# xipengwang/AprilSAM

Measured on AMD Instinct MI355X. Metric: Gauss-Newton iterations/sec + factorise ms on M3500 (chi2 match <=1e-6), higher is better.
Workload: dtype f64; 1 GPU; M3500 batch april_graph_cholesky, 1 replica per GPU (3500 poses, 5454 factors, n=10500); parallelism=single GPU, fronts=680, levels=9, nnz_L=422121

## Files before the change

### aprilsam_amd/csrc/kernels.hip.h

```cpp
#pragma once
#include <hip/hip_runtime.h>
#include <stdint.h>

#include <type_traits>
namespace asam {

constexpr int PROF_SLOTS = 16;
constexpr int PROF_XCD_UP = 12, PROF_XCD_DN = 13;
constexpr int PROF_X_STORED = 14, PROF_X_DRAINED = 11, PROF_X_FLAG = 15;
constexpr int PROF_EA_ISSUED = 8, PROF_EA_DATA = 9, PROF_EA_ADDS = 10, PROF_EA_REST = 14, PROF_EA_END = 15;
#ifdef APRILSAM_AMD_EA_STAMPS
constexpr bool EA_STAMPS = true;
#else
constexpr bool EA_STAMPS = false;
#endif
__device__ __forceinline__ int xcc_id() { return __builtin_amdgcn_s_getreg(20 | (0 << 6) | ((4 - 1) << 11)) & 7; }
constexpr int TPB = 256;
constexpr int NB = 32;
constexpr int TILE = 64;
constexpr int ASM_CB = 4;
constexpr int OBP = 4;

struct FrontDesc {
    long long off;
    int nsb, nub, first;
    int dest_begin, dest_end;
    int ch_begin, ch_end;
    int rows_begin;
    int parent;
    int dinv0;
    int prim1, prim2;
    int own_nw;
    int pad;
};
static_assert(sizeof(FrontDesc) == 64, "FrontDesc must stay one cache line");
struct DestRec { int brow, bcol, src_begin, src_end; };
struct ChildRec {
    long long uoff;
    int cR;
    int cnu;
    int rel_begin;
    int pad;
};
static_assert(sizeof(ChildRec) == 24, "ChildRec layout");

struct DevPlan {
    int nF;
    const FrontDesc *fd;
    const DestRec *dest;
    const ChildRec *child;
    const int *f_rows, *f_rel;
    const int *f_own; int own_lo, own_hi;
    const int *slot_blk, *slot_rhs;
    const int *src_idx;
    const double *lambda;
    long long *prof;
    int prof_mode;
    int schur_first_nub;
    int *epoch; const int *flevel; int l0; const int *marks;
    int xmode; uint4 *xg; unsigned xg_bytes;
};
enum { X_FLUSH = 0, X_WT = 1, X_TAGGED = 2 };
constexpr int XG_CONST = -1;

__host__ __device__ inline int asm_chunks(int nbc) { return (nbc + ASM_CB - 1) / ASM_CB; }
struct SyrkRange { int k_lo, k_hi, col_lo, col_hi, ntr, ntc; };
__host__ __device__ inline SyrkRange syrk_range(int R, int C, int ns, int s_lo, int s_hi, int tile = TILE, bool ahead = false) {
    SyrkRange g;
    g.k_lo = s_lo * NB;
    g.k_hi = s_hi * NB < ns ? s_hi * NB : ns;
    g.col_lo = g.k_hi;
    g.col_hi = ahead ? (g.k_hi + OBP * NB < ns ? g.k_hi + OBP * NB : ns) : C;
    if (g.k_hi <= g.k_lo || g.col_hi <= g.col_lo) { g.ntr = g.ntc = 0; return g; }
    g.ntr = ((R - 2) - g.col_lo + tile - 1) / tile;
    g.ntc = (g.col_hi - g.col_lo + tile - 1) / tile;
    return g;
}
__host__ __device__ inline int syrk_tiles(int R, int C, int ns, int s_lo, int s_hi, int tile = TILE, bool ahead = false) {
    SyrkRange g = syrk_range(R, C, ns, s_lo, s_hi, tile, ahead);
    return g.ntc * g.ntr - g.ntc * (g.ntc - 1) / 2;
}
__device__ __forceinline__ int find_seg(const int *__restrict__ pre, int n, int bid) {
    int lo = 0, hi = n;
    while (hi - lo > 1) { int m = (lo + hi) >> 1; if (pre[m] <= bid) lo = m; else hi = m; }
    return lo;
}

__device__ __forceinline__ void trapezoid_tile(int l, int ntr, int ntc, int *ti, int *tj_);
constexpr int SYRK_SB = 8;
constexpr int SYRK_MODE_XCD_SHIFT = 8;
__host__ __device__ inline void trapezoid_tile_xcd(int l, int nt, int ntr, int ntc, int *ti, int *tj) {
// ... 742 lines not shown
    for (int l = wave; l < ntiles; l += nw) {
        int ti = l, tj = 0;
        while (ti >= ntr - tj) { ti -= ntr - tj; tj++; }
        ti += tj;
        const int i0 = col_lo + 16 * ti, j0 = col_lo + 16 * tj;
        const int rj = min(j0 + l15, Rv - 1), ri = min(i0 + l15, Rv - 1);
        const int i = i0 + l15, jb = j0 + l4;
        const int cbase = jb * ld + i;
        bool ok[4];
#pragma unroll
        for (int reg = 0; reg < 4; reg++) { const int j = jb + 4 * reg; ok[reg] = i < Rv && j < col_hi && i >= j; }
        double cv[4], x[4], y[4];
#pragma unroll
        for (int reg = 0; reg < 4; reg++) cv[reg] = S[ok[reg] ? cbase + 4 * reg * ld : 0];
#pragma unroll
        for (int ks = 0; ks < 4; ks++) {
            const int kk = 4 * ks + l4;
            const double *col = S + (k_lo + (kk < kw ? kk : 0)) * ld;
            x[ks] = col[rj]; y[ks] = col[ri];
        }
        d4_t acc = (d4_t){ 0, 0, 0, 0 };
#pragma unroll
        for (int ks = 0; ks < 4; ks++) {
            if (ks < nk) {
                const bool kok = 4 * ks + l4 < kw;
                acc = __builtin_amdgcn_mfma_f64_16x16x4f64(kok ? x[ks] : 0.0, kok ? y[ks] : 0.0, acc, 0, 0, 0);
            }
        }
#pragma unroll
        for (int reg = 0; reg < 4; reg++) if (ok[reg]) S[cbase + 4 * reg * ld] = cv[reg] - acc[reg];
    }
}

constexpr int GB = 4;

constexpr int BW = 16;
template <int NT, int BWT>
__device__ __forceinline__ void chain_block(double *S, int ld, int k0, int wdt, int Rv, int *bad, double (&Dd)[BWT], int nwc) {
    constexpr int BROWS = 64 - BWT;
    constexpr int PER = BWT <= 8 ? 1 : (BWT - 2 + 7) / 8;
    const int wave = __builtin_amdgcn_readfirstlane(threadIdx.x >> 6), lane = threadIdx.x & 63;
    const bool isdiag = lane < BWT;
    const int below0 = k0 + wdt;
    const int nchunk = max(1, (Rv - below0 + BROWS - 1) / BROWS);
    if (wave >= nchunk) return;
    for (int ch = wave + ((nchunk - 1 - wave) / nwc) * nwc; ch >= wave; ch -= nwc) {
        const int row = isdiag ? k0 + lane : below0 + BROWS * ch + (lane - BWT);
        const bool valid = isdiag ? lane < wdt : row < Rv;
        const int rowc = valid ? row : k0;
        double D[BWT];
#pragma unroll
        for (int c = 0; c < BWT; c++) D[c] = S[(size_t)(k0 + (c < wdt ? c : 0)) * ld + rowc];
        int isbad = 0;
        double dn = readlane_d(D[0], 0);
        if (!(dn > 0)) isbad = 1;
        double inv = fast_rsqrt(dn);
#pragma unroll
        for (int j = 0; j < BWT; j++) {
            D[j] *= inv;
            double lc[BWT];
            if (j + 1 < BWT) {
                lc[j + 1] = readlane_d(D[j], j + 1);
                D[j + 1] = fma(-D[j], lc[j + 1], D[j + 1]);
                dn = readlane_d(D[j + 1], j + 1);
                if (j + 1 < wdt && !(dn > 0)) isbad = 1;
            }
// ... 8 lines not shown
                    else if (st == 1 || st == 4) e = -h * y;
                    else if (st == 2 || st == 5) e = fma(e, y, 0.5);
                    else if (st == 3 || st == 6) y = fma(y, e, y);
                }
#pragma unroll
                for (int q = 0; q < PER; q++) {
                    const int c = j + 2 + PER * st + q;
                    if (c < BWT) D[c] = fma(-D[j], lc[c], D[c]);
                }
                __builtin_amdgcn_sched_barrier(0);
            }
            inv = y;
        }
        if (valid && !isdiag) {
#pragma unroll
            for (int c = BWT - 1; c >= 0; c--) S[(size_t)(k0 + (c < wdt ? c : 0)) * ld + row] = (c < wdt) ? D[c] : D[0];
        }
        if (ch == 0) {
#pragma unroll
            for (int c = 0; c < BWT; c++) Dd[c] = D[c];
            if (isbad && lane == 0) { if (atomicCAS(bad, 0, 1) == 0) { bad[2] = 1; bad[3] = k0 / 3; } }
        }
    }
}
template <int BWT>
__device__ __forceinline__ void chain_store_diag(double *S, int ld, int k0, int wdt, const double (&Dd)[BWT]) {
    const int r = threadIdx.x & 63;
    if (r < wdt) {
#pragma unroll
        for (int c = 0; c < BWT; c++) if (c < wdt) S[(k0 + c) * ld + k0 + r] = (c <= r) ? Dd[c] : 0.0;
    }
}
template <int NT>
__device__ __forceinline__ void factor_dense_blk(double *S, int ld, int ns, int Rv, int hi, int *bad, double * , long long *pf = nullptr) {
    constexpr int NW = NT / 64;
    long long t_chain = 0, t_syrk = 0, t0 = 0;
    const int wave = __builtin_amdgcn_readfirstlane(threadIdx.x >> 6);
    auto chain_sync_store = [&](int k0, int nwc) {
        const int wdt = min(BW, ns - k0);
        if (wdt <= 8) {
            double D8[8];
            chain_block<NT, 8>(S, ld, k0, wdt, Rv, bad, D8, nwc);
            __syncthreads();
            if (wave == 0) chain_store_diag<8>(S, ld, k0, wdt, D8);
        } else {
            double D16[16];
            chain_block<NT, 16>(S, ld, k0, wdt, Rv, bad, D16, nwc);
            __syncthreads();
            if (wave == 0) chain_store_diag<16>(S, ld, k0, wdt, D16);
        }
    };
    auto chain_waves = [&](int k0) {
        const int wdt = min(BW, ns - k0), brows = 64 - (wdt <= 8 ? 8 : 16);
        const int nchunk = max(1, (Rv - (k0 + wdt) + brows - 1) / brows);
        return min(nchunk, NW / 2);
    };
    if (pf) t0 = wall_clock64();
    chain_sync_store(0, NW);
    if (pf) { const long long t1 = wall_clock64(); t_chain += t1 - t0; t0 = t1; }
    for (int k0 = 0; k0 < ns; k0 += BW) {
        const int wdt = min(BW, ns - k0), below0 = k0 + wdt;
        if (below0 < ns) {
            const int next_hi = min(below0 + BW, ns), cw = chain_waves(below0);
            if (NW >= 8) lds_syrk16<NT>(S, ld, k0, below0, below0, next_hi, Rv, 1, NW - 1);
            else lds_syrk16<NT>(S, ld, k0, below0, below0, next_hi, Rv);
            __syncthreads();
            if (pf) { const long long t1 = wall_clock64(); t_syrk += t1 - t0; t0 = t1; }
            if (wave < cw) {
                long long w0_ = 0, c0_ = 0;
                if (pf) { w0_ = wall_clock64(); c0_ = clock64(); }
                chain_sync_store(below0, cw);
                if (pf && threadIdx.x == 0) { pf[10] += clock64() - c0_; pf[15] += wall_clock64() - w0_; }
            } else {
                if (next_hi < hi) lds_syrk16<NT>(S, ld, k0, below0, next_hi, hi, Rv, cw, NW - cw);
                __syncthreads();
            }
            if (pf) { const long long t1 = wall_clock64(); t_chain += t1 - t0; t0 = t1; }
        } else {
            __syncthreads();
            if (below0 < hi) lds_syrk16<NT>(S, ld, k0, below0, below0, hi, Rv);
            __syncthreads();
            if (pf) { const long long t1 = wall_clock64(); t_syrk += t1 - t0; t0 = t1; }
        }
    }
    if (pf && threadIdx.x == 0) { pf[8] = t_chain; pf[9] = t_syrk; }
}
template <int NT>
__device__ __forceinline__ void factor_front_blk(double *S, int ld, int nsb, int nbc, int *bad, double *stage, int nbc_upd = -1, long long *pf = nullptr) {
    if (nbc_upd < 0) nbc_upd = nbc;
    factor_dense_blk<NT>(S, ld, 3 * nsb, 3 * (nbc + 1) - 2, 3 * nbc_upd, bad, stage, pf);
}

__host__ __device__ inline size_t small_front_lds(int R, int C, int nw) { return (size_t)(R | 1) * C * 8 + wl_bytes(nw); }
__host__ __device__ inline size_t panel_front_lds(int R, int ns, int nw) { return (size_t)(R | 1) * ns * 8 + wl_bytes(nw); }
__host__ __device__ inline bool front_runs_full(int R, int C, int nw, long long full_lds_limit) { return (long long)small_front_lds(R, C, nw) <= full_lds_limit; }

template <int NT>
__device__ __forceinline__ void front_small_body(const DevPlan &P, const int t, double *__restrict__ pool, const double *__restrict__ Hc, int *bad,
                                                 long long full_lds_limit, int *flags, int wait, double *S) {
    const int *wflags = wait ? flags : nullptr;
    const int ev = flags ? flag_value(P) : 0;
    const FrontDesc D = P.fd[t];
    const int nsb = D.nsb, nbc = D.nsb + D.nub;
    const int R = 3 * (nbc + 1), C = 3 * nbc, ld = R | 1;
    double *Fg = pool + D.off;
    if (P.prof && threadIdx.x == 0) P.prof[(size_t)t * PROF_SLOTS + PROF_XCD_UP] = 1 + xcc_id();
    if (front_runs_full(R, C, NT / 64, full_lds_limit)) {
        int2 *wl = (int2 *)(S + (size_t)ld * C);
        if (P.prof && threadIdx.x == 0) P.prof[(size_t)t * PROF_SLOTS + 0] = wall_clock64();
        assemble_front<NT, ASM_LDS>(P, D, pool, Hc, 0, nbc, true, S, ld, nullptr, 0, wl, P.prof ? P.prof + (size_t)t * PROF_SLOTS : nullptr, wflags, bad, ev);
        if (P.prof && threadIdx.x == 0) P.prof[(size_t)t * PROF_SLOTS + 1] = wall_clock64();
        factor_front_blk<NT>(S, ld, nsb, nbc, bad, (double *)wl, -1, (P.prof && (!EA_STAMPS || P.prof_mode < 4)) ? P.prof + (size_t)t * PROF_SLOTS : nullptr);
        if (P.prof && threadIdx.x == 0) P.prof[(size_t)t * PROF_SLOTS + 2] = wall_clock64();
        for (int c = 3 * nsb + (threadIdx.x >> 6); c < C; c += NT / 64) {
            int r0 = 3 * (c / 3);
            for (int r = r0 + (threadIdx.x & 63); r < R; r += 64) Fg[(size_t)c * R + r] = S[(size_t)c * ld + r];
        }
        if (flags) publish_flag(flags + t, ev);
        for (int c = threadIdx.x >> 6; c < 3 * nsb; c += NT / 64) {
            int r0 = 3 * (c / 3);
            for (int r = r0 + (threadIdx.x & 63); r < R; r += 64) Fg[(size_t)c * R + r] = S[(size_t)c * ld + r];
        }
    } else {
        const int ns = 3 * nsb;
        int2 *wl = (int2 *)(S + (size_t)ld * ns);
        const bool schur_first = P.schur_first_nub > 0 && D.nub >= P.schur_first_nub;
        if (P.prof && threadIdx.x == 0) P.prof[(size_t)t * PROF_SLOTS + 0] = wall_clock64();
        if (schur_first) assemble_front<NT, ASM_SPLIT>(P, D, pool, Hc, 0, nsb, false, S, ld, Fg, R, wl, P.prof ? P.prof + (size_t)t * PROF_SLOTS : nullptr, wflags, bad, ev);
        else assemble_front<NT, ASM_SPLIT>(P, D, pool, Hc, 0, nbc, true, S, ld, Fg, R, wl, P.prof ? P.prof + (size_t)t * PROF_SLOTS : nullptr, wflags, bad, ev);
        if (P.prof && threadIdx.x == 0) P.prof[(size_t)t * PROF_SLOTS + 1] = wall_clock64();
        factor_front_blk<NT>(S, ld, nsb, nbc, bad, (double *)wl, nsb, (P.prof && (!EA_STAMPS || P.prof_mode < 4)) ? P.prof + (size_t)t * PROF_SLOTS : nullptr);
        if (P.prof && threadIdx.x == 0) P.prof[(size_t)t * PROF_SLOTS + 2] = wall_clock64();
        if (schur_first) {
            lds_panel_syrk<NT, 2>(S, ld, 0, ns, ns, C, R - 2, Fg, R);
            __syncthreads();
            assemble_front<NT, ASM_GLOBAL, false>(P, D, pool, Hc, nsb, nbc, false, nullptr, 0, Fg, R, wl, nullptr, nullptr, bad);
        }
        else if (nbc > nsb) lds_panel_syrk<NT, 1>(S, ld, 0, ns, ns, C, R - 2, Fg, R);
        if (flags) publish_flag(flags + t, ev);
        for (int c = threadIdx.x >> 6; c < ns; c += NT / 64) {
            int r0 = 3 * (c / 3);
            for (int r = r0 + (threadIdx.x & 63); r < R; r += 64) Fg[(size_t)c * R + r] = S[(size_t)c * ld + r];
        }
    }
    if (P.prof) { __syncthreads(); if (threadIdx.x == 0) P.prof[(size_t)t * PROF_SLOTS + 3] = wall_clock64(); }
}
constexpr int UPD_MAXF = 4;
constexpr int UPD_MAXC = 4;
struct UpdRec {
    long long old_off;
    int mode;
    int old_nub;
    int wout;
    int mask;
    int n_own, own_f[UPD_MAXF], own_la[UPD_MAXF], own_lb[UPD_MAXF], own_slot[UPD_MAXF];
    int n_ch, ch_t[UPD_MAXC], ch_wout[UPD_MAXC], ch_rel[UPD_MAXC], ch_cnu[UPD_MAXC], ch_mask[UPD_MAXC];
    int pad[3];
};
static_assert(sizeof(UpdRec) == 192, "UpdRec layout");
struct UpdCtx {
    const UpdRec *recs;
    double *wbuf;
    int *wflags;
    const int *fa, *fb; const double *Z, *Wm, *lp, *st;
};
__host__ __device__ inline size_t update_front_lds(int R, int ns, int nact) {
    return (size_t)((size_t)ns * (R | 1) + (size_t)3 * nact * (R | 1) + 8 * ns + 3 * (ns | 1) + 16) * 8;
}
template <int NT>
__device__ __forceinline__ void front_update_body(const DevPlan &P, const int t, const UpdRec &rec, const UpdCtx &uc, double *__restrict__ pool,
                                                  int *flags, int *bad, double *S) {
    constexpr int NW = NT / 64;
// ... 1580 lines not shown
```

### aprilsam_amd/csrc/solver.h

```cpp
#pragma once
#include <vector>
#include "../../include/aprilsam_amd.h"

namespace asam {

struct Options {
    int leaf_nodes = 16;
    int deterministic = 0;
    int use_graph = 1;
    int device_timing = 0;
    int trust_factor_cache = 0;
    int small_lds_kb = 156;
    int inc_fast = 1;
    int inc_multi = 1;
    int inc_one = 1;
    int inc_one_up = 3, inc_one_dn = 4, inc_one_threads = 512, inc_one_spin = 1;
    int inc_tail = 1;
    int inc_inline = 1;
    int inc_tail_solve = 1;
    int inc_lazy_states = 1;
    int inc_replan_tall = 1;
    int inc_update = 1;
    int speculate_factors = 1;
    int warm_up = 1;
    int syrk_xcd_order = 512;
    int syrk_small_tiles = 320;
    int syrk_pair_tiles = 2048;
    int syrk_group = 3;
    int schur_first = 40;
    int small_threads = 1024;
    int tp_threads = 512;
    int tp_fronts = 1000;
    int tp_lds_kb = 80;
    int amalg = 0;
    int amalg_max = 64;
    int pin_last = 0;
    int batch_extend = 1;
    int extend_tail_fronts = 3;
    int persist = 1;
    int persist_max_fronts = 240;
    int persist_leaves = 1;
    int persist_up = 2;
    int xcd_place = 1;
    int asm_balance = 1;
    int tail_poses = 28;
    int blk_backsolve = 1;
    int wave_backsolve = 1;
    int tagged_x = 1;
    int linearize_staged_min = 32768;
    int mem_cap_mb = 0;
    int solve_chunk_cols = 0;
    int pool_guard = 0;
    int pool_poison = 0;
    int skip_flag_waits = 0;
    int polar_on_host = 0;
    int gaussian_on_host = 0;
    int panel_mode = 1;
};
extern Options g_opt;

void batch_step(april_graph_t *g, april_graph_cholesky_param_t *param);
void inc_step(april_graph_t *g, april_graph_cholesky_param_t *param);
void inc_solve_only(april_graph_t *g, april_graph_cholesky_param_t *param);
double graph_chi2(april_graph_t *g);
int batch_resident(april_graph_t *g, april_graph_cholesky_param_t *param, int iters, double *chi2_out, double *ms_out);
int resident_begin(april_graph_t *g, april_graph_cholesky_param_t *param);
int resident_steps(april_graph_t *g, april_graph_cholesky_param_t *param, int n, int mode);
int resident_sync(april_graph_t *g, april_graph_cholesky_param_t *param);
double resident_chi2(april_graph_t *g);
int resident_end(april_graph_t *g, april_graph_cholesky_param_t *param);
int level_profile(const april_graph_cholesky_param_t *param, double *out, int cap_levels);
int debug_front_forms(const april_graph_cholesky_param_t *param, int *out, int cap);
int debug_inc_forms(const april_graph_cholesky_param_t *param, int *out, int cap);
int kernel_profile(const april_graph_cholesky_param_t *param, double *ms, long long *calls, double *flops, double *bytes, const char **names);
void drop_context(const april_graph_cholesky_param_t *p);
void drop_graph_pack(const april_graph_t *g);
bool get_stats(const april_graph_cholesky_param_t *p, aprilsam_amd_stats_t *out);
// ... 73 lines not shown
```

### aprilsam_amd/csrc/solver.hip.cpp

```cpp
#include <hip/hip_runtime.h>
#include <rccl/rccl.h>
#include <dlfcn.h>

#include <algorithm>
#include <array>
#include <chrono>
#include <thread>
#include <cmath>
#include <cstdarg>
#include <cstdio>
#include <cstdlib>
#include <cstring>
#include <functional>
#include <map>
#include <memory>
#include <atomic>
#include <mutex>
#include <string>
#include <unordered_map>
#include <vector>

#include "../../include/aprilsam_amd.h"
#include "errors.h"
#include "kernels.hip.h"
// ... 19 lines not shown

#define HIPCHECK(expr)                                                                                 \
    do {                                                                                               \
        hipError_t e_ = (expr);                                                                        \
        if (e_ != hipSuccess) {                                                                        \
            (void)hipGetLastError();                                                                   \
            fail(e_ == hipErrorOutOfMemory ? ERR_OOM : ERR_HIP, "%s failed: %s (%s:%d)", #expr, hipGetErrorString(e_), __FILE__, __LINE__); \
        }                                                                                              \
    } while (0)

static double now_ms() {
    return std::chrono::duration<double, std::milli>(std::chrono::steady_clock::now().time_since_epoch()).count();
}

Options g_opt;
struct OptionDef { const char *name; int Options::*member; int min_value; bool policy; int max_value = 0x7fffffff; };
static const OptionDef OPTION_TABLE[] = {
    { "leaf_nodes", &Options::leaf_nodes, 1, false }, { "deterministic", &Options::deterministic, 0, true }, { "use_graph", &Options::use_graph, 0, true },
    { "device_timing", &Options::device_timing, 0, true }, { "trust_factor_cache", &Options::trust_factor_cache, 0, true },
    { "small_lds_kb", &Options::small_lds_kb, 0, false }, { "syrk_xcd_order", &Options::syrk_xcd_order, 0, false },
    { "schur_first", &Options::schur_first, 0, false }, { "syrk_small_tiles", &Options::syrk_small_tiles, 0, false }, { "syrk_pair_tiles", &Options::syrk_pair_tiles, 0, false }, { "syrk_group", &Options::syrk_group, 2, false, 8 }, { "panel_mode", &Options::panel_mode, 0, false },
    { "small_threads", &Options::small_threads, 64, false }, { "tp_fronts", &Options::tp_fronts, 0, false }, { "tp_lds_kb", &Options::tp_lds_kb, 0, false },
    { "tp_threads", &Options::tp_threads, 64, false }, { "inc_fast", &Options::inc_fast, 0, true }, { "inc_multi", &Options::inc_multi, 0, true },
    { "inc_one", &Options::inc_one, 0, true }, { "inc_one_up", &Options::inc_one_up, 1, true }, { "inc_one_dn", &Options::inc_one_dn, 1, true },
    { "inc_one_threads", &Options::inc_one_threads, 64, true }, { "inc_one_spin", &Options::inc_one_spin, 0, true }, { "inc_tail", &Options::inc_tail, 0, false },
    { "inc_inline", &Options::inc_inline, 0, true }, { "inc_update", &Options::inc_update, 0, true }, { "inc_tail_solve", &Options::inc_tail_solve, 0, true },
    { "inc_lazy_states", &Options::inc_lazy_states, 0, true }, { "inc_replan_tall", &Options::inc_replan_tall, 0, true },
    { "speculate_factors", &Options::speculate_factors, 0, true }, { "warm_up", &Options::warm_up, 0, true }, { "pin_last", &Options::pin_last, 0, false }, { "persist", &Options::persist, 0, false },
    { "persist_max_fronts", &Options::persist_max_fronts, 0, false }, { "xcd_place", &Options::xcd_place, 0, false }, { "persist_leaves", &Options::persist_leaves, 0, false, 1 }, { "persist_up", &Options::persist_up, 0, false, 3 }, { "linearize_staged_min", &Options::linearize_staged_min, 0, false },
    { "wave_backsolve", &Options::wave_backsolve, 0, false }, { "tagged_x", &Options::tagged_x, 0, false, 2 }, { "blk_backsolve", &Options::blk_backsolve, 0, false }, { "tail_poses", &Options::tail_poses, 8, false },
    { "batch_extend", &Options::batch_extend, 0, true }, { "extend_tail_fronts", &Options::extend_tail_fronts, 0, true }, { "mem_cap_mb", &Options::mem_cap_mb, 0, true }, { "solve_chunk_cols", &Options::solve_chunk_cols, 0, true },
    { "pool_guard", &Options::pool_guard, 0, false }, { "amalg", &Options::amalg, 0, false }, { "amalg_max", &Options::amalg_max, 1, false }, { "pool_poison", &Options::pool_poison, 0, false }, { "skip_flag_waits", &Options::skip_flag_waits, 0, false },
    { "polar_on_host", &Options::polar_on_host, 0, false, 1 }, { "gaussian_on_host", &Options::gaussian_on_host, 0, false, 1 }, { "asm_balance", &Options::asm_balance, 0, false, 1 },
};
static const OptionDef *find_option(const char *name) {
    for (const OptionDef &d : OPTION_TABLE) if (!strcmp(d.name, name)) return &d;
    return nullptr;
}
static std::once_flag g_opt_once;
static void load_env_options() {
    std::call_once(g_opt_once, [] {
        for (const OptionDef &d : OPTION_TABLE) {
            std::string env = "APRILSAM_AMD_";
            for (const char *q = d.name; *q; q++) env += (char)toupper((unsigned char)*q);
            const char *sv = getenv(env.c_str());
            if (sv && *sv) g_opt.*(d.member) = std::min(d.max_value, std::max(d.min_value, (int)atof(sv)));
        }
    });
}

constexpr int MAX_SLOTS = 64;
static std::atomic<int> g_device{ -1 };
static std::mutex g_slot_mu[MAX_SLOTS];
static thread_local int t_slot = 0;
static int device_count() {
    static std::atomic<int> cached{ 0 };
    int n = cached.load(std::memory_order_relaxed);
    if (n > 0) return n;
    if (hipGetDeviceCount(&n) != hipSuccess) { (void)hipGetLastError(); return 0; }
    if (n > 0) cached.store(n, std::memory_order_relaxed);
    return n;
}
static int physical_device(int slot) { const int n = device_count(); return n > 0 ? slot % n : 0; }
static thread_local int t_device = -1;
template <class V> struct Registry {
    using Map = std::map<const void *, std::unique_ptr<V>>;
// ... 413 lines not shown
```

### aprilsam_amd/csrc/solver_context.inc.h

```cpp
enum { K_LINEARIZE = 0, K_FRONT_SMALL, K_ASSEMBLE_BIG, K_PANEL_BIG, K_SYRK_BIG, K_BACKSOLVE, K_UPDATE, NKERN };
static const char *const KNAMES[NKERN] = { "k_linearize", "k_front_small", "k_assemble_big", "k_panel_big", "k_syrk_big", "k_backsolve", "k_update_states" };
struct Launch { int list_off, pre_off, n, grid; bool single = false; int tile = TILE; };

struct LevelPlan {
    int small_off = 0, n_small = 0; size_t small_lds = 0;
    long long full_limit = 0;
    int small_nt = 512;
    int n_big = 0; size_t asm_lds = 0;
    Launch asm_big{};
    std::vector<Launch> syrka, syrk1;
    bool paired = false;
    std::vector<Launch> bchain, btile, syrkw;
    int all_off = 0, n_all = 0; size_t solve_lds = 0;
    size_t solve_w_lds = 0; int maxns = 0;
    Launch bs_gemv{};
    Launch bs_blk{}; size_t bs_blk_lds = 0;
    int rest_off = 0, n_rest = 0; size_t rest_lds = 0;
};

struct IncState {
    bool ready = false;
    bool pristine = false;
    int Nb = 0, Fb = 0, nF0 = 0, nLev0 = 0;
    int cap_nodes = 0, cap_fact = 0;
// ... 507 lines not shown
    const double u1 = uprof ? now_ms() : 0;
    const bool inc = c.want_inc;
    const int INC_NODES_ = inc ? INC_NODES : 0, INC_FACT_ = inc ? INC_FACT : 0;
    const size_t INC_I32_ = inc ? INC_I32 : 0, INC_DEST_ = inc ? INC_DEST : 0, INC_CHILD_ = inc ? INC_CHILD : 0, INC_TAB_ = inc ? INC_TAB : 0;
    c.inc.cap_nodes = INC_NODES_; c.inc.cap_fact = INC_FACT_;
    std::vector<int> i32;
    auto put32 = [&](const std::vector<int> &v) { size_t o = i32.size(); i32.insert(i32.end(), v.begin(), v.end()); if (v.empty()) i32.push_back(0); return o; };
    size_t o_rows = put32(P.f_rows), o_rel = put32(P.f_rel);
    const bool own_tab = g_opt.asm_balance && !lay && !P.f_rel.empty();
    const size_t o_own = own_tab ? put32(std::vector<int>(P.f_rel.size(), -1)) : 0;
    size_t o_sb = put32(P.slot_blk); i32.resize(i32.size() + (size_t)3 * INC_FACT_, -1);
    size_t o_sr = put32(P.slot_rhs); i32.resize(i32.size() + (size_t)2 * INC_FACT_, -1);
    c.inc.i32_used = (long long)i32.size(); c.inc.dest_used = (long long)P.dest.size(); c.inc.child_used = (long long)P.ch_idx.size();
    for (int t = 0; t < P.nF; t++) fd[t].rows_begin = (int)(o_rows + P.f_rows_ptr[t]);
    for (size_t k = 0; k < P.ch_idx.size(); k++) ch[k].rel_begin = (int)(o_rel + P.f_rows_ptr[ch[k].pad]);
    c.d_i32.need(i32.size() + INC_I32_); c.d_fd.need(fd.size() + 1 + (inc ? MAX_TAIL_FRONTS : 0)); c.d_child.need(ch.size() + INC_CHILD_);
    c.d_dest.need(std::max<size_t>(1, P.dest.size()) + INC_DEST_);
    HIPCHECK(hipMemcpyAsync(c.d_i32.p, i32.data(), i32.size() * 4, hipMemcpyHostToDevice, s));
    HIPCHECK(hipMemcpyAsync(c.d_fd.p, fd.data(), fd.size() * sizeof(FrontDesc), hipMemcpyHostToDevice, s));
    HIPCHECK(hipMemcpyAsync(c.d_child.p, ch.data(), ch.size() * sizeof(ChildRec), hipMemcpyHostToDevice, s));
    static_assert(sizeof(DestRec) == sizeof(Plan::DestRec), "DestRec layout");
    if (!P.dest.empty()) HIPCHECK(hipMemcpyAsync(c.d_dest.p, P.dest.data(), P.dest.size() * sizeof(DestRec), hipMemcpyHostToDevice, s));
    c.d_lambda.need((size_t)P.N + INC_NODES_);
    DevPlan &d = c.dp;
    d.nF = P.nF;
    d.fd = c.d_fd.p; d.dest = c.d_dest.p; d.child = c.d_child.p;
    d.f_own = nullptr; d.own_lo = 0; d.own_hi = 0;
    if (own_tab) { d.f_own = c.d_i32.p + o_own - o_rel; d.own_lo = (int)o_rel; d.own_hi = (int)(o_rel + P.f_rel.size()); }
    d.f_rows = c.d_i32.p; d.f_rel = c.d_i32.p; d.slot_blk = c.d_i32.p + o_sb; d.slot_rhs = c.d_i32.p + o_sr; d.src_idx = c.d_i32.p;
    c.inc.o_rows = (long long)o_rows; c.inc.o_rel = (long long)o_rel;
    d.lambda = c.d_lambda.p;
    d.prof = nullptr; d.prof_mode = 0;
    d.schur_first_nub = std::max(0, g_opt.schur_first);
    d.epoch = nullptr; d.flevel = nullptr; d.l0 = 0; d.marks = nullptr;
    if (getenv("APRILSAM_AMD_KPROF")) { c.d_prof.need((size_t)PROF_SLOTS * P.nF); HIPCHECK(hipMemsetAsync(c.d_prof.p, 0, (size_t)8 * PROF_SLOTS * P.nF, s)); d.prof = c.d_prof.p; d.prof_mode = atoi(getenv("APRILSAM_AMD_KPROF")) >= 2 ? atoi(getenv("APRILSAM_AMD_KPROF")) : 1; }
    c.d_swap.need((size_t)P.F + INC_FACT_); c.d_pos.need((size_t)P.N + INC_NODES_);
    fill_swap_host(c);
    HIPCHECK(hipMemcpyAsync(c.d_swap.p, c.swap_host.data(), P.F, hipMemcpyHostToDevice, s));
    c.wt_dirty = false;
    HIPCHECK(hipMemcpyAsync(c.d_pos.p, P.pos.data(), (size_t)P.N * 4, hipMemcpyHostToDevice, s));
    c.d_perm.need((size_t)P.N + INC_NODES_);
    HIPCHECK(hipMemcpyAsync(c.d_perm.p, P.perm.data(), (size_t)P.N * 4, hipMemcpyHostToDevice, s));

    const double u2 = uprof ? now_ms() : 0;
    std::vector<int> tab;
    c.levels.assign(P.nLevels, LevelPlan());
    for (int l = 0; l < P.nLevels; l++) {
        std::vector<int> fr(P.lev_fronts.begin() + P.lev_ptr[l], P.lev_fronts.begin() + P.lev_ptr[l + 1]);
        build_level(c.levels[l], fr, tab, [&](int t, int *nsb, int *nub) { *nsb = P.f_nsb[t]; *nub = P.f_nub[t]; }, [](int) { return true; });
    }
    if (own_tab) {
        std::vector<int> own(P.f_rel.size(), -1);
        for (int l = 0; l < P.nLevels; l++) {
            const LevelPlan &L = c.levels[l];
            for (int k = 0; k < L.n_small; k++) {
                const int t = tab[L.small_off + k];
                if (P.ch_ptr[t + 1] == P.ch_ptr[t]) continue;
                fd[t].own_nw = waves_of(L.small_nt);
                asm_owners(P.f_nsb[t] + P.f_nub[t], fd[t].own_nw, P.ch_idx.data() + P.ch_ptr[t], P.ch_ptr[t + 1] - P.ch_ptr[t], P.f_rows_ptr.data(), P.f_nub.data(), P.f_rel.data(), own.data());
            }
        }
        HIPCHECK(hipMemcpyAsync(c.d_i32.p + o_own, own.data(), own.size() * 4, hipMemcpyHostToDevice, s));
    }
    {
        long long slots = 0;
        for (int t = 0; t < P.nF; t++) fd[t].dinv0 = -1;
// ... 241 lines not shown
```

### aprilsam_amd/csrc/solver_resident.inc.h

```cpp
static int resident_begin_impl(april_graph_t *g, april_graph_cholesky_param_t *param);
int resident_begin(april_graph_t *g, april_graph_cholesky_param_t *param) { return guarded_rc(param, g, [&] { return resident_begin_impl(g, param); }); }
static int resident_begin_impl(april_graph_t *g, april_graph_cholesky_param_t *param) {
    if (zsize(g->nodes) == 0 || zsize(g->factors) == 0) return -1;
    ensure_device();
    SlotLock lk(param, g);
    Context &c = ctx_for(param);
    GraphPack &gp = pack_for(g);
    pack_factors(gp, g);
    if (!gp.host_idx.empty()) return -4;
    pack_states(gp, g, false);
    sync_fixed(gp, g);
    gp.lp_last_valid = false;
    orient_asymmetric(c, gp);
    const bool reused = prepare_plan(c, gp, g);
    flush_orientation(c, gp.stream);
    upload_factors(gp);
    upload_fixed(gp);
    set_lambda(c, gp, param->tikhanov);
    if (!c.have_events) { for (auto &e : c.ev) HIPCHECK(hipEventCreate(&e)); c.have_events = true; }
    for (int k = 0; k < NKERN; k++) { c.k_ms[k] = 0; c.k_calls[k] = 0; }
    c.lev_up_ms.clear(); c.lev_dn_ms.clear();
    c.st.n_nodes = gp.N; c.st.n_factors = gp.F; c.st.symbolic_reused = reused; c.st.not_spd = 0; c.st.error_code = 0;
    c.resident_failed = false; c.resident_stepped = false;
    HIPCHECK(hipStreamSynchronize(gp.stream));
// ... 223 lines not shown
        if (small) { flops[K_FRONT_SMALL] += fl; bytes[K_FRONT_SMALL] += by; }
        else {
            const double Rv = R - 2;
            double fsy = 0;
            auto trapezoid = [&](double c_lo, double c_hi) { const double n = c_hi - c_lo; return n <= 0 ? 0.0 : n * Rv - (c_lo + c_hi - 1) * n / 2; };
            const int steps = ((int)ns + NB - 1) / NB;
            for (int o = 0; o * OBP < steps; o++) {
                const double k_lo = (double)o * OBP * NB, k_hi = std::min<double>(ns, (double)(o + 1) * OBP * NB);
                fsy += 2.0 * (k_hi - k_lo) * trapezoid(k_hi, C);
            }
            fsy = std::min(fsy, fl);
            flops[K_SYRK_BIG] += fsy; flops[K_PANEL_BIG] += fl - fsy;
            bytes[K_SYRK_BIG] += by; bytes[K_ASSEMBLE_BIG] += by;
        }
        bytes[K_BACKSOLVE] += 8.0 * (ns * (ns + 1) / 2 + nu * ns) + 16.0 * (ns + nu);
        flops[K_BACKSOLVE] += 2.0 * (ns * (ns + 1) / 2 + nu * ns);
    }
    int F2 = 0, F1 = 0;
    for (int f = 0; f < P.F; f++) (c.pat[2 * f + 1] >= 0 ? F2 : F1)++;
    bytes[K_LINEARIZE] = F2 * 152.0 + F1 * 124.0 + 8.0 * (27.0 * F2 + 9.0 * F1 + 6.0 * F2 + 3.0 * F1);
    flops[K_LINEARIZE] = 150.0 * F2 + 40.0 * F1;
    bytes[K_UPDATE] = 8.0 * 3 * P.N * 4;
    return NKERN;
}

static int debug_stage_impl(april_graph_t *g, april_graph_cholesky_param_t *param, int what, double *out);
int debug_stage(april_graph_t *g, april_graph_cholesky_param_t *param, int what, double *out) { return guarded_rc(param, g, [&] { return debug_stage_impl(g, param, what, out); }); }
static int debug_stage_impl(april_graph_t *g, april_graph_cholesky_param_t *param, int what, double *out) {
    if (zsize(g->nodes) == 0 || zsize(g->factors) == 0) return -1;
    ensure_device();
    SlotLock lk(param, g);
    Context &c = ctx_for(param);
    GraphPack &gp = pack_for(g);
    pack_factors(gp, g);
    if (!gp.host_idx.empty()) return -4;
    pack_states(gp, g, false);
    sync_fixed(gp, g);
    orient_asymmetric(c, gp);
    prepare_plan(c, gp, g);
    flush_orientation(c, gp.stream);
    upload_factors(gp);
    upload_fixed(gp);
    const Plan &P = c.plan;
    const int N = gp.N, F = gp.F;
    hipStream_t s = gp.stream;
    gp.mirror_sync = false;
    HIPCHECK(hipMemcpyAsync(gp.d_lp.p, gp.d_state.p, (size_t)24 * N, hipMemcpyDeviceToDevice, s));
    enqueue_families_before(gp, s, nullptr);
    hipLaunchKernelGGL((k_linearize_t<false>), dim3((F + TPB - 1) / TPB), dim3(TPB), 0, s, 0, F, (const int *)nullptr, gp.d_fa.p, gp.d_fb.p, gp.d_z.p, gp.d_W.p,
                       gp.d_lp.p, gp.d_state.p, c.d_swap.p, c.dp.slot_blk, c.dp.slot_rhs, c.d_H.p, c.d_bad.p, (const double *)nullptr);
    if (gp.n_fixed() > 0) {
        set_lambda(c, gp, param->tikhanov);
        c.lambda_N = -1;
    }
    enqueue_families_after(c, gp, s);
    if (what == 0) {
        std::vector<double> H((size_t)9 * std::max(1, P.n_slots));
        HIPCHECK(hipMemcpyAsync(H.data(), c.d_H.p, H.size() * 8, hipMemcpyDeviceToHost, s));
        HIPCHECK(hipStreamSynchronize(s));
        for (int f = 0; f < F; f++) {
            double *o = out + (size_t)33 * f;
            memset(o, 0, 33 * 8);
            memcpy(o, &H[(size_t)9 * P.slot_blk[3 * f]], 72);
            memcpy(o + 27, &H[(size_t)9 * P.slot_rhs[2 * f]], 24);
            if (gp.h_fb.p[f] < 0) continue;
            const double *b1 = &H[(size_t)9 * P.slot_blk[3 * f + 1]];
// ... 51 lines not shown
```

Before: 5597 GN iterations/s.

## Fuse front Schur-complement tail update with global store of update block

Adds a front_tail mode, on by default, in which the final SYRK pass over a front's update columns writes results straight to the global front pool instead of back to LDS followed by a separate copy loop. During the last chain step, the idle waves compute up to TAIL_HOLD tiles of the trailing update, keep them in registers, and finish and store them to global once the last panel is ready. The remaining tiles go out in the final pass, and a few extra entries are stored ahead of time. This removes the LDS round trip and the copy-out loop on the critical path, at the cost of more register pressure and a new debug dump path for checking correctness.

```diff
diff --git a/aprilsam_amd/csrc/kernels.hip.h b/aprilsam_amd/csrc/kernels.hip.h
--- a/aprilsam_amd/csrc/kernels.hip.h
+++ b/aprilsam_amd/csrc/kernels.hip.h
@@ -6,6 +6,7 @@
 namespace asam {
 
 constexpr int PROF_SLOTS = 16;
+constexpr int PROF_TAIL_PASS = 13, PROF_TAIL_FLAG = 14;
 constexpr int PROF_XCD_UP = 12, PROF_XCD_DN = 13;
 constexpr int PROF_X_STORED = 14, PROF_X_DRAINED = 11, PROF_X_FLAG = 15;
 constexpr int PROF_EA_ISSUED = 8, PROF_EA_DATA = 9, PROF_EA_ADDS = 10, PROF_EA_REST = 14, PROF_EA_END = 15;
@@ -57,6 +58,7 @@
     long long *prof;
     int prof_mode;
     int schur_first_nub;
+    int front_tail;
     int *epoch; const int *flevel; int l0; const int *marks;
     int xmode; uint4 *xg; unsigned xg_bytes;
 };
@@ -865,6 +867,112 @@
     }
 }
 
+constexpr int TAIL_HOLD = 4;
+struct Syrk16Tile { int cbase, gbase, rj, ri; bool ok[4]; };
+__device__ __forceinline__ Syrk16Tile syrk16_tile(int l, int ld, int ldg, int col_lo, int col_hi, int Rv) {
+    const int lane = threadIdx.x & 63, l15 = lane & 15, l4 = lane >> 4;
+    const int ntr = (Rv - col_lo + 15) >> 4;
+    int ti = l, tj = 0;
+    while (ti >= ntr - tj) { ti -= ntr - tj; tj++; }
+    ti += tj;
+    const int i0 = col_lo + 16 * ti, j0 = col_lo + 16 * tj;
+    Syrk16Tile T;
+    T.rj = min(j0 + l15, Rv - 1); T.ri = min(i0 + l15, Rv - 1);
+    const int i = i0 + l15, jb = j0 + l4;
+    T.cbase = jb * ld + i; T.gbase = jb * ldg + i;
+#pragma unroll
+    for (int reg = 0; reg < 4; reg++) { const int j = jb + 4 * reg; T.ok[reg] = i < Rv && j < col_hi && i >= j; }
+    return T;
+}
+__device__ __forceinline__ int syrk16_ntiles(int col_lo, int col_hi, int Rv) {
+    const int ntr = (Rv - col_lo + 15) >> 4, ntc = (col_hi - col_lo + 15) >> 4;
+    return ntc * ntr - ntc * (ntc - 1) / 2;
+}
+__device__ __forceinline__ d4_t syrk16_product(const double *__restrict__ S, int ld, int k_lo, int k_hi, const Syrk16Tile &T) {
+    const int l4 = (threadIdx.x & 63) >> 4;
+    const int kw = k_hi - k_lo, nk = (kw + 3) >> 2;
+    double x[4], y[4];
+#pragma unroll
+    for (int ks = 0; ks < 4; ks++) {
+        const int kk = 4 * ks + l4;
+        const double *col = S + (k_lo + (kk < kw ? kk : 0)) * ld;
+        x[ks] = col[T.rj]; y[ks] = col[T.ri];
+    }
+    d4_t acc = (d4_t){ 0, 0, 0, 0 };
+#pragma unroll
+    for (int ks = 0; ks < 4; ks++) {
+        if (ks < nk) {
+            const bool kok = 4 * ks + l4 < kw;
+            acc = __builtin_amdgcn_mfma_f64_16x16x4f64(kok ? x[ks] : 0.0, kok ? y[ks] : 0.0, acc, 0, 0, 0);
+        }
+    }
+    return acc;
+}
+template <int NT>
+__device__ __forceinline__ void lds_syrk16_out(const double *__restrict__ S, int ld, int k_lo, int k_hi, int col_lo, int col_hi, int Rv,
+                                               double *__restrict__ Cg, int ldg, int l_lo) {
+    const int wave = __builtin_amdgcn_readfirstlane((int)(threadIdx.x >> 6));
+    const int ntiles = syrk16_ntiles(col_lo, col_hi, Rv);
+    for (int l = l_lo + wave; l < ntiles; l += NT / 64) {
+        const Syrk16Tile T = syrk16_tile(l, ld, ldg, col_lo, col_hi, Rv);
+        double cv[4];
+#pragma unroll
+        for (int reg = 0; reg < 4; reg++) cv[reg] = S[T.ok[reg] ? T.cbase + 4 * reg * ld : 0];
+        const d4_t acc = syrk16_product(S, ld, k_lo, k_hi, T);
+#pragma unroll
+        for (int reg = 0; reg < 4; reg++) if (T.ok[reg]) Cg[(size_t)T.gbase + (size_t)(4 * reg) * ldg] = cv[reg] - acc[reg];
+    }
+}
+template <int NT>
+__device__ __forceinline__ void lds_syrk16_hold_out(double *__restrict__ S, int ld, int kp_lo, int kp_hi, int kl_hi, int col_lo, int col_hi, int Rv,
+                                                    int w0, double *__restrict__ Cg, int ldg) {
+    const int nw = NT / 64 - w0;
+    const int wave = __builtin_amdgcn_readfirstlane((int)(threadIdx.x >> 6)) - w0;
+    const int ntiles = syrk16_ntiles(col_lo, col_hi, Rv);
+    d4_t held[TAIL_HOLD];
+#pragma unroll
+    for (int m = 0; m < TAIL_HOLD; m++) {
+        const int l = wave + m * nw;
+        if (l < ntiles) {
+            const Syrk16Tile T = syrk16_tile(l, ld, ldg, col_lo, col_hi, Rv);
+            double cv[4];
+#pragma unroll
+            for (int reg = 0; reg < 4; reg++) cv[reg] = S[T.ok[reg] ? T.cbase + 4 * reg * ld : 0];
+            const d4_t acc = syrk16_product(S, ld, kp_lo, kp_hi, T);
+#pragma unroll
+            for (int reg = 0; reg < 4; reg++) held[m][reg] = cv[reg] - acc[reg];
+        }
+    }
+    for (int l = wave + TAIL_HOLD * nw; l < ntiles; l += nw) {
+        const Syrk16Tile T = syrk16_tile(l, ld, ldg, col_lo, col_hi, Rv);
+        double cv[4];
+#pragma unroll
+        for (int reg = 0; reg < 4; reg++) cv[reg] = S[T.ok[reg] ? T.cbase + 4 * reg * ld : 0];
+        const d4_t acc = syrk16_product(S, ld, kp_lo, kp_hi, T);
+#pragma unroll
+        for (int reg = 0; reg < 4; reg++) if (T.ok[reg]) S[T.cbase + 4 * reg * ld] = cv[reg] - acc[reg];
+    }
+    __syncthreads();
+#pragma unroll
+    for (int m = 0; m < TAIL_HOLD; m++) {
+        const int l = wave + m * nw;
+        if (l < ntiles) {
+            const Syrk16Tile T = syrk16_tile(l, ld, ldg, col_lo, col_hi, Rv);
+            const d4_t acc = syrk16_product(S, ld, kp_hi, kl_hi, T);
+#pragma unroll
+            for (int reg = 0; reg < 4; reg++) if (T.ok[reg]) Cg[(size_t)T.gbase + (size_t)(4 * reg) * ldg] = held[m][reg] - acc[reg];
+        }
+    }
+}
+template <int NT>
+__device__ __forceinline__ void store_tail_extras(const double *__restrict__ S, int ld, double *__restrict__ Fg, int R, int ns, int C) {
+    for (int e = threadIdx.x; e < 4 * (C - ns); e += NT) {
+        const int c = ns + (e >> 2), q = e & 3;
+        const int r = q < 2 ? 3 * (c / 3) + q : R - 4 + q;
+        if (q >= 2 || r < c) Fg[(size_t)c * R + r] = S[(size_t)c * ld + r];
+    }
+}
+
 constexpr int GB = 4;
 
 constexpr int BW = 16;
@@ -939,9 +1047,11 @@
     }
 }
 template <int NT>
-__device__ __forceinline__ void factor_dense_blk(double *S, int ld, int ns, int Rv, int hi, int *bad, double * , long long *pf = nullptr) {
+__device__ __forceinline__ void factor_dense_blk(double *S, int ld, int ns, int Rv, int hi, int *bad, double * , long long *pf = nullptr,
+                                                 int tail = 0, double *Fg = nullptr, int ldg = 0) {
     constexpr int NW = NT / 64;
     long long t_chain = 0, t_syrk = 0, t0 = 0;
+    int l_out = 0;
     const int wave = __builtin_amdgcn_readfirstlane(threadIdx.x >> 6);
     auto chain_sync_store = [&](int k0, int nwc) {
         const int wdt = min(BW, ns - k0);
@@ -973,18 +1083,27 @@
             else lds_syrk16<NT>(S, ld, k0, below0, below0, next_hi, Rv);
             __syncthreads();
             if (pf) { const long long t1 = wall_clock64(); t_syrk += t1 - t0; t0 = t1; }
+            const bool fuse = tail && Fg && next_hi == ns && ns < hi;
+            if (fuse) l_out = TAIL_HOLD * (NW - cw);
             if (wave < cw) {
                 long long w0_ = 0, c0_ = 0;
                 if (pf) { w0_ = wall_clock64(); c0_ = clock64(); }
                 chain_sync_store(below0, cw);
                 if (pf && threadIdx.x == 0) { pf[10] += clock64() - c0_; pf[15] += wall_clock64() - w0_; }
+            } else if (fuse) {
+                lds_syrk16_hold_out<NT>(S, ld, k0, below0, ns, ns, hi, Rv, cw, Fg, ldg);
             } else {
                 if (next_hi < hi) lds_syrk16<NT>(S, ld, k0, below0, next_hi, hi, Rv, cw, NW - cw);
                 __syncthreads();
             }
             if (pf) { const long long t1 = wall_clock64(); t_chain += t1 - t0; t0 = t1; }
+        } else if (tail) {
+            if (pf && threadIdx.x == 0) pf[PROF_TAIL_PASS] = wall_clock64();
+            if (below0 < hi && Fg) lds_syrk16_out<NT>(S, ld, k0, below0, below0, hi, Rv, Fg, ldg, l_out);
+            if (pf) { const long long t1 = wall_clock64(); t_syrk += t1 - t0; t0 = t1; }
         } else {
             __syncthreads();
+            if (pf && threadIdx.x == 0) pf[PROF_TAIL_PASS] = wall_clock64();
             if (below0 < hi) lds_syrk16<NT>(S, ld, k0, below0, below0, hi, Rv);
             __syncthreads();
             if (pf) { const long long t1 = wall_clock64(); t_syrk += t1 - t0; t0 = t1; }
@@ -993,9 +1112,10 @@
     if (pf && threadIdx.x == 0) { pf[8] = t_chain; pf[9] = t_syrk; }
 }
 template <int NT>
-__device__ __forceinline__ void factor_front_blk(double *S, int ld, int nsb, int nbc, int *bad, double *stage, int nbc_upd = -1, long long *pf = nullptr) {
+__device__ __forceinline__ void factor_front_blk(double *S, int ld, int nsb, int nbc, int *bad, double *stage, int nbc_upd = -1, long long *pf = nullptr,
+                                                 int tail = 0, double *Fg = nullptr) {
     if (nbc_upd < 0) nbc_upd = nbc;
-    factor_dense_blk<NT>(S, ld, 3 * nsb, 3 * (nbc + 1) - 2, 3 * nbc_upd, bad, stage, pf);
+    factor_dense_blk<NT>(S, ld, 3 * nsb, 3 * (nbc + 1) - 2, 3 * nbc_upd, bad, stage, pf, tail, Fg, 3 * (nbc + 1));
 }
 
 __host__ __device__ inline size_t small_front_lds(int R, int C, int nw) { return (size_t)(R | 1) * C * 8 + wl_bytes(nw); }
@@ -1011,19 +1131,25 @@
     const int nsb = D.nsb, nbc = D.nsb + D.nub;
     const int R = 3 * (nbc + 1), C = 3 * nbc, ld = R | 1;
     double *Fg = pool + D.off;
+    const int tail = P.front_tail;
     if (P.prof && threadIdx.x == 0) P.prof[(size_t)t * PROF_SLOTS + PROF_XCD_UP] = 1 + xcc_id();
     if (front_runs_full(R, C, NT / 64, full_lds_limit)) {
         int2 *wl = (int2 *)(S + (size_t)ld * C);
         if (P.prof && threadIdx.x == 0) P.prof[(size_t)t * PROF_SLOTS + 0] = wall_clock64();
         assemble_front<NT, ASM_LDS>(P, D, pool, Hc, 0, nbc, true, S, ld, nullptr, 0, wl, P.prof ? P.prof + (size_t)t * PROF_SLOTS : nullptr, wflags, bad, ev);
         if (P.prof && threadIdx.x == 0) P.prof[(size_t)t * PROF_SLOTS + 1] = wall_clock64();
-        factor_front_blk<NT>(S, ld, nsb, nbc, bad, (double *)wl, -1, (P.prof && (!EA_STAMPS || P.prof_mode < 4)) ? P.prof + (size_t)t * PROF_SLOTS : nullptr);
+        if (tail) store_tail_extras<NT>(S, ld, Fg, R, 3 * nsb, C);
+        factor_front_blk<NT>(S, ld, nsb, nbc, bad, (double *)wl, -1, (P.prof && (!EA_STAMPS || P.prof_mode < 4)) ? P.prof + (size_t)t * PROF_SLOTS : nullptr, tail, Fg);
         if (P.prof && threadIdx.x == 0) P.prof[(size_t)t * PROF_SLOTS + 2] = wall_clock64();
-        for (int c = 3 * nsb + (threadIdx.x >> 6); c < C; c += NT / 64) {
-            int r0 = 3 * (c / 3);
-            for (int r = r0 + (threadIdx.x & 63); r < R; r += 64) Fg[(size_t)c * R + r] = S[(size_t)c * ld + r];
+        if (!tail) {
+            for (int c = 3 * nsb + (threadIdx.x >> 6); c < C; c += NT / 64) {
+                int r0 = 3 * (c / 3);
+                for (int r = r0 + (threadIdx.x & 63); r < R; r += 64) Fg[(size_t)c * R + r] = S[(size_t)c * ld + r];
+            }
         }
         if (flags) publish_flag(flags + t, ev);
+        else if (tail) __syncthreads();
+        if (P.prof && P.prof_mode == 1 && threadIdx.x == 0) P.prof[(size_t)t * PROF_SLOTS + PROF_TAIL_FLAG] = wall_clock64();
         for (int c = threadIdx.x >> 6; c < 3 * nsb; c += NT / 64) {
             int r0 = 3 * (c / 3);
             for (int r = r0 + (threadIdx.x & 63); r < R; r += 64) Fg[(size_t)c * R + r] = S[(size_t)c * ld + r];
@@ -1036,7 +1162,7 @@
         if (schur_first) assemble_front<NT, ASM_SPLIT>(P, D, pool, Hc, 0, nsb, false, S, ld, Fg, R, wl, P.prof ? P.prof + (size_t)t * PROF_SLOTS : nullptr, wflags, bad, ev);
         else assemble_front<NT, ASM_SPLIT>(P, D, pool, Hc, 0, nbc, true, S, ld, Fg, R, wl, P.prof ? P.prof + (size_t)t * PROF_SLOTS : nullptr, wflags, bad, ev);
         if (P.prof && threadIdx.x == 0) P.prof[(size_t)t * PROF_SLOTS + 1] = wall_clock64();
-        factor_front_blk<NT>(S, ld, nsb, nbc, bad, (double *)wl, nsb, (P.prof && (!EA_STAMPS || P.prof_mode < 4)) ? P.prof + (size_t)t * PROF_SLOTS : nullptr);
+        factor_front_blk<NT>(S, ld, nsb, nbc, bad, (double *)wl, nsb, (P.prof && (!EA_STAMPS || P.prof_mode < 4)) ? P.prof + (size_t)t * PROF_SLOTS : nullptr, tail);
         if (P.prof && threadIdx.x == 0) P.prof[(size_t)t * PROF_SLOTS + 2] = wall_clock64();
         if (schur_first) {
             lds_panel_syrk<NT, 2>(S, ld, 0, ns, ns, C, R - 2, Fg, R);
@@ -1045,6 +1171,8 @@
         }
         else if (nbc > nsb) lds_panel_syrk<NT, 1>(S, ld, 0, ns, ns, C, R - 2, Fg, R);
         if (flags) publish_flag(flags + t, ev);
+        else if (tail) __syncthreads();
+        if (P.prof && P.prof_mode == 1 && threadIdx.x == 0) P.prof[(size_t)t * PROF_SLOTS + PROF_TAIL_FLAG] = wall_clock64();
         for (int c = threadIdx.x >> 6; c < ns; c += NT / 64) {
             int r0 = 3 * (c / 3);
             for (int r = r0 + (threadIdx.x & 63); r < R; r += 64) Fg[(size_t)c * R + r] = S[(size_t)c * ld + r];
diff --git a/aprilsam_amd/csrc/solver.h b/aprilsam_amd/csrc/solver.h
--- a/aprilsam_amd/csrc/solver.h
+++ b/aprilsam_amd/csrc/solver.h
@@ -43,6 +43,7 @@
     int persist_up = 2;
     int xcd_place = 1;
     int asm_balance = 1;
+    int front_tail = 1;
     int tail_poses = 28;
     int blk_backsolve = 1;
     int wave_backsolve = 1;
diff --git a/aprilsam_amd/csrc/solver.hip.cpp b/aprilsam_amd/csrc/solver.hip.cpp
--- a/aprilsam_amd/csrc/solver.hip.cpp
+++ b/aprilsam_amd/csrc/solver.hip.cpp
@@ -75,6 +75,7 @@
     { "batch_extend", &Options::batch_extend, 0, true }, { "extend_tail_fronts", &Options::extend_tail_fronts, 0, true }, { "mem_cap_mb", &Options::mem_cap_mb, 0, true }, { "solve_chunk_cols", &Options::solve_chunk_cols, 0, true },
     { "pool_guard", &Options::pool_guard, 0, false }, { "amalg", &Options::amalg, 0, false }, { "amalg_max", &Options::amalg_max, 1, false }, { "pool_poison", &Options::pool_poison, 0, false }, { "skip_flag_waits", &Options::skip_flag_waits, 0, false },
     { "polar_on_host", &Options::polar_on_host, 0, false, 1 }, { "gaussian_on_host", &Options::gaussian_on_host, 0, false, 1 }, { "asm_balance", &Options::asm_balance, 0, false, 1 },
+    { "front_tail", &Options::front_tail, 0, false, 1 },
 };
 static const OptionDef *find_option(const char *name) {
     for (const OptionDef &d : OPTION_TABLE) if (!strcmp(d.name, name)) return &d;
diff --git a/aprilsam_amd/csrc/solver_context.inc.h b/aprilsam_amd/csrc/solver_context.inc.h
--- a/aprilsam_amd/csrc/solver_context.inc.h
+++ b/aprilsam_amd/csrc/solver_context.inc.h
@@ -563,6 +563,7 @@
     d.lambda = c.d_lambda.p;
     d.prof = nullptr; d.prof_mode = 0;
     d.schur_first_nub = std::max(0, g_opt.schur_first);
+    d.front_tail = g_opt.front_tail ? 1 : 0;
     d.epoch = nullptr; d.flevel = nullptr; d.l0 = 0; d.marks = nullptr;
     if (getenv("APRILSAM_AMD_KPROF")) { c.d_prof.need((size_t)PROF_SLOTS * P.nF); HIPCHECK(hipMemsetAsync(c.d_prof.p, 0, (size_t)8 * PROF_SLOTS * P.nF, s)); d.prof = c.d_prof.p; d.prof_mode = atoi(getenv("APRILSAM_AMD_KPROF")) >= 2 ? atoi(getenv("APRILSAM_AMD_KPROF")) : 1; }
     c.d_swap.need((size_t)P.F + INC_FACT_); c.d_pos.need((size_t)P.N + INC_NODES_);
diff --git a/aprilsam_amd/csrc/solver_resident.inc.h b/aprilsam_amd/csrc/solver_resident.inc.h
--- a/aprilsam_amd/csrc/solver_resident.inc.h
+++ b/aprilsam_amd/csrc/solver_resident.inc.h
@@ -279,6 +279,22 @@
     SlotLock lk(param, g);
     Context &c = ctx_for(param);
     GraphPack &gp = pack_for(g);
+    if (what == 2) {
+        const Plan &P = c.plan;
+        if (P.nF <= 0 || !c.d_pool.p || (long long)c.d_pool.cap < (long long)P.pool_doubles) return -3;
+        std::vector<double> pool((size_t)P.pool_doubles);
+        HIPCHECK(hipStreamSynchronize(gp.stream));
+        HIPCHECK(hipMemcpy(pool.data(), c.d_pool.p, pool.size() * 8, hipMemcpyDeviceToHost));
+        memset(out, 0, pool.size() * 8);
+        for (int t = 0; t < P.nF; t++) {
+            const int nbc = P.f_nsb[t] + P.f_nub[t], R = 3 * (nbc + 1);
+            for (int col = 0; col < 3 * nbc; col++) {
+                const size_t o = (size_t)P.f_off[t] + (size_t)col * R + 3 * (col / 3);
+                memcpy(out + o, pool.data() + o, (size_t)(R - 3 * (col / 3)) * 8);
+            }
+        }
+        return 0;
+    }
     pack_factors(gp, g);
     if (!gp.host_idx.empty()) return -4;
     pack_states(gp, g, false);
```

Result: no change. 5640 GN iterations/s (median of 6 runs) (+0.8%).
